# daisy9542/yolo-puncture

Hardware: AMD Instinct MI355X
Metric: images/sec (higher is better)
Workload: dtype bf16

## Files before the change

### include/yolop.h

```cpp
#ifndef YOLOP_H
#define YOLOP_H

#include <stddef.h>
#include <stdint.h>

#ifdef __cplusplus
extern "C" {
#endif

#define YP_OK 0
#define YP_ERR_ARG -1
#define YP_ERR_STATE -2
#define YP_ERR_HIP -3
#define YP_ERR_WEIGHT -4

#define YP_BF16 0
#define YP_F32 1

#define YP_TASK_DETECT 0
#define YP_TASK_SEGMENT 1

#define YP_NM 32
#define YP_MAX_MASKS 480
#define YP_ID_MASKS_FRAMES_BUDGET (1ull << 30)
// ... 121 lines not shown
int yp_tensor_write(yp_engine* e, int tensor, int coff, int C, const float* host);
int yp_tensor_count(const yp_engine* e);
int yp_tensor_info(const yp_engine* e, int i, char* name, int name_cap, int dims[4] , int* is_f32);
int yp_tensor_read(yp_engine* e, int i, float* host_out);

int yp_profile(yp_engine* e, const uint8_t* in_dev, int B, int H, int W, float* det_out, int32_t* idx_out,
               float* coeff_out, float* ms_out, int iters, void* stream);

int yp_set_nms(yp_engine* e, float conf, float iou);

int yp_set_attention_form(yp_engine* e, int form);

int yp_set_attention_f32_stream(yp_engine* e, int on);

int yp_set_autotune(yp_engine* e, int enable);

int yp_tuning_export(const yp_engine* e, int32_t* cfg_out, int cap);
int yp_tuning_import(yp_engine* e, int B, int H, int W, const int32_t* cfg, int n);

int yp_debug_force_conv_cfg(int cfg);
int yp_debug_op_cfg(const yp_engine* e, int i, int* cfg);
int yp_debug_last_store_form(void);
int yp_debug_max_workgroups(int n);
int yp_debug_conv_families(int* base, int* num_cfgs, int cap);
int yp_debug_ablation(int v);
int yp_debug_head_clocks(uint64_t* out8);
int yp_debug_attention(const void* qkv_dev, void* o_dev, int dtype, int B, int N, int nh, int kd, int hd, int q_stride, int q_coff, int o_stride,
                       int o_coff, int wgs, int* kernel_out, void* stream);
int yp_debug_attention_form(const void* qkv_dev, void* o_dev, int dtype, int B, int N, int nh, int kd, int hd, int q_stride, int q_coff, int o_stride,
                            int o_coff, int wgs, int form, int* kernel_out, void* stream);
int yp_debug_attention_f32(const void* qkv_dev, void* o_dev, int B, int N, int nh, int kd, int hd, int q_stride, int q_coff, int o_stride, int o_coff,
                           int wgs, int f32_stream, int* kernel_out, void* stream);
int yp_debug_conv_s2(const void* x_dev, const void* w_dev, const float* bias_dev, const void* res_dev, void* y_dev, int out_f32, int B, int H,
                     int W, int Cin, int Cout, int silu, int cfg, int lds_weights, int64_t* lds_out, char* kernel_out, int kernel_cap,
                     void* stream);
int yp_debug_topk_anchors(const uint32_t* const mk_dev[3], int B, const int hw[3][2], int k, int32_t* sel_out_dev, uint32_t* thr_out_dev, void* stream);
int yp_debug_head_branch_clocks(uint64_t* out8);
int yp_debug_head_winners(yp_engine* e, int32_t* sel_host, float* box_host, float* coeff_host);
int yp_debug_contour_clocks(uint64_t* out12);
int yp_debug_pwsp_clocks(uint64_t* out32);

int yp_tuning_source(const yp_engine* e);

int yp_debug_host_selftest(yp_engine* e);
int yp_debug_graph_info(const yp_engine* e, int64_t* out6);
int yp_debug_head_positions(yp_engine* e, int64_t* out6);
// ... 9 lines not shown
```

### yolo-puncture_amd/csrc/common.h

```cpp
#pragma once
#include <hip/hip_runtime.h>
#include <stdint.h>
#include <atomic>
#include <cstdlib>
#include <initializer_list>
#include <string>
#include <type_traits>
#include <vector>

namespace yp {

enum DType { DT_BF16 = 0, DT_F32 = 1 };
enum Act { ACT_NONE = 0, ACT_SILU = 1, ACT_RELU = 2 };

enum OpKind {
    OP_STEM = 0,
    OP_CONV = 1,
    OP_DWCONV = 2,
    OP_POOL5 = 3,
    OP_UPSAMPLE = 4,
    OP_ATTN = 5,
    OP_HEAD = 6,
    OP_CONVT = 7,
    OP_AMAX = 9,
// ... 106 lines not shown
    void* y; int y_stride, y_coff; int Ho, Wo;
    const void* res; int res_stride, res_coff;
    int B, ks, stride, pad, act;
    int gs, gstride;
    size_t x_bytes;
};

struct StemParams {
    const uint8_t* x; int H, W;
    const float* w;
    const void* wpk;
    const float* bias;
    void* y; int y_stride, y_coff; int Ho, Wo, C0; int B;
    int act;
};

struct FrontParams {
    const uint8_t* img; int imgH, imgW, B;
    const void* w0; const float* bias0; int act0, C0; int H1, W1;
    const void* w1; const float* bias1; int act1, C1, Kpad1; size_t w1_bytes;
    const void* w2; const float* bias2; int act2, C2, Kpad2; size_t w2_bytes;
    void* y; int y_stride, y_coff; size_t y_bytes; int Ho, Wo;
    unsigned long long* clk;
};
bool frontend_valid(const FrontParams& p);
hipError_t launch_frontend(const FrontParams& p, hipStream_t st);

struct C2fParams {
    const void* x; int x_stride, x_coff; size_t x_bytes;
    int B, H, W, C;
    const void* w1; const float* bias1; int act1, Kpad1; size_t w1_bytes;
    const void* w2; const float* bias2; int act2, Kpad2; size_t w2_bytes;
    int shortcut;
    const void* w3; const float* bias3; int act3, Kpad3, Cout; size_t w3_bytes;
    void* y; int y_stride, y_coff; size_t y_bytes;
    unsigned long long* clk;
    int wide;
};
bool c2f_fused_valid(const C2fParams& p);

struct ScdParams {
    const void* x; int x_stride, x_coff; size_t x_bytes; int B, H, W, K;
    const void* w1; const float* bias1; int act1, Kpad1, C; size_t w1_bytes;
    const void* wd; const float* biasd; int actd;
    void* y; int y_stride, y_coff; size_t y_bytes; int Ho, Wo;
    unsigned long long* clk;
};
bool scdown_fused_valid(const ScdParams& p);
// ... 313 lines not shown
```

### yolo-puncture_amd/csrc/engine.hip

```cpp
#include "../../include/yolop.h"
#include "common.h"
#include <algorithm>
#include <array>
#include <chrono>

#include <cmath>
#include <cstdarg>
#include <cstdio>
#include <cstring>
#include <cstdlib>
#include <dlfcn.h>
#include <fcntl.h>
#include <fstream>
#include <map>
#include <sstream>
#include <memory>

using namespace yp;

static thread_local char g_err[512] = "";
static int fail(int code, const char* fmt, ...) {
    va_list ap;
    va_start(ap, fmt);
    vsnprintf(g_err, sizeof(g_err), fmt, ap);
// ... 9 lines not shown

struct yp_engine {
    yp_model_desc desc{};
    int device = 0;
    int dtype = DT_BF16;
    std::vector<TensorDesc> tensors;
    std::vector<WeightDesc> weights;
    std::vector<Op> ops;
    std::map<std::string, int> wmap;
    bool finalized = false;
    int pB = 0, pH = 0, pW = 0;
    bool planned = false, allocated = false;
    void* arena = nullptr;
    size_t arena_bytes = 0;
    int proto_t = -1;
    void* mask_ws = nullptr;
    void* head_ws = nullptr;
    size_t head_ws_bytes = 0;
    size_t mask_ws_bytes = 0;
    bool use_graph = false;
    bool graph_auto = false;
    std::map<std::array<int, 3>, bool> auto_replay;
    bool fuse = true;
    int attn_form = ATTN_FORM_AUTO;
    int attn_f32_stream = ATTN_F32_GENERIC;
    bool tail = false;
    bool narrow_store = false;
    bool sparse_head = true;
    void* sp_ws = nullptr; size_t sp_ws_bytes = 0;
    bool tune = true;
    int tune_source = 0;
    hipStream_t own_stream = nullptr;
    hipEvent_t ev_in = nullptr;
    hipGraphExec_t gexec = nullptr;
    hipGraph_t gsrc = nullptr;
    bool use_lanes = true;
    int n_captures = 0;
    int g_nodes = 0, g_edges = 0, g_edges_expected = 0;
    hipStream_t last_stream = nullptr; bool have_last = false;
    struct LaneStep { int op = -1; std::vector<int> waits; bool fork = false; bool record = false; };
    std::vector<LaneStep> lane_steps;
    std::vector<int> lanes_used;
    int n_lanes = 1;
    bool warmed = false;
    struct Tuned { int cfg; std::string kernel; };
    std::map<std::array<int, 3>, std::vector<Tuned>> tuned;
// ... 587 lines not shown
    p.out_f32 = (to.f32 && e.dtype == DT_BF16) ? 1 : 0;
    p.wide = (e.dtype == DT_BF16 && !p.out_f32 && !e.narrow_store) ? 1 : 0;
    p.up = 1; p.oy = 0; p.ox = 0;
    p.x_bytes = ti.bytes; p.w_bytes = w.mat_bytes; p.y_bytes = to.bytes; p.cfg = o.cfg; p.dbg = conv_debug_ablation();
    if (o.folded) {
        const Op& u = e.ops[o.fold_up];
        const TensorDesc& t2 = e.tensors[u.in.t];
        p.x2 = t2.ptr; p.x2_bytes = t2.bytes; p.x2_stride = t2.C; p.x2_coff = u.in.coff; p.x2_C = u.out.C; p.x2_H = t2.H; p.x2_W = t2.W;
    }
    return p;
}

static FrontParams front_params(const yp_engine& e, const Op& o, const uint8_t* img) {
    const Op& c1 = e.ops[o.fuse_pre];
    const Op& st = e.ops[o.stem_op];
    const WeightDesc &w0 = e.weights[st.widx], &w1 = e.weights[c1.widx], &w2 = e.weights[o.widx];
    const TensorDesc &t0 = e.tensors[st.out.t], &to = e.tensors[o.out.t];
    FrontParams p{};
    p.img = img; p.imgH = e.pH; p.imgW = e.pW; p.B = e.pB;
    p.w0 = w0.d_w2; p.bias0 = w0.d_b; p.act0 = st.act; p.C0 = st.out.C; p.H1 = t0.H; p.W1 = t0.W;
    p.w1 = w1.d_w; p.bias1 = w1.d_b; p.act1 = c1.act; p.C1 = c1.out.C; p.Kpad1 = w1.Kpad; p.w1_bytes = w1.mat_bytes;
    p.w2 = w2.d_w; p.bias2 = w2.d_b; p.act2 = o.act; p.C2 = o.out.C; p.Kpad2 = w2.Kpad; p.w2_bytes = w2.mat_bytes;
    p.y = to.ptr; p.y_stride = to.C; p.y_coff = o.out.coff; p.y_bytes = to.bytes; p.Ho = to.H; p.Wo = to.W;
    return p;
}

static C2fParams c2f_params(const yp_engine& e, const Op& o) {
    const Op &m1 = e.ops[o.c2f_m1], &m2 = e.ops[o.c2f_m2];
    const WeightDesc &w1 = e.weights[m1.widx], &w2 = e.weights[m2.widx], &w3 = e.weights[o.widx];
    const TensorDesc &ti = e.tensors[o.in.t], &to = e.tensors[o.out.t];
    C2fParams p{};
    p.x = ti.ptr; p.x_stride = ti.C; p.x_coff = o.in.coff; p.x_bytes = ti.bytes; p.B = e.pB; p.H = ti.H; p.W = ti.W; p.C = m1.in.C;
    p.w1 = w1.d_w; p.bias1 = w1.d_b; p.act1 = m1.act; p.Kpad1 = w1.Kpad; p.w1_bytes = w1.mat_bytes;
    p.w2 = w2.d_w; p.bias2 = w2.d_b; p.act2 = m2.act; p.Kpad2 = w2.Kpad; p.w2_bytes = w2.mat_bytes;
    p.shortcut = m2.res.t >= 0 ? 1 : 0;
    p.w3 = w3.d_w; p.bias3 = w3.d_b; p.act3 = o.act; p.Kpad3 = w3.Kpad; p.Cout = o.out.C; p.w3_bytes = w3.mat_bytes;
    p.y = to.ptr; p.y_stride = to.C; p.y_coff = o.out.coff; p.y_bytes = to.bytes;
    p.wide = (e.dtype == DT_BF16 && !to.f32 && !e.narrow_store) ? 1 : 0;
    if (m1.in.t != o.in.t || m1.in.coff != o.in.coff + p.C || m2.out.t != o.in.t || m2.out.coff != o.in.coff + 2 * p.C || o.in.C != 3 * p.C ||
        m1.k != 3 || m2.k != 3 || m1.s != 1 || m2.s != 1 || m1.out.C != p.C || m2.out.C != p.C || m1.res.t >= 0 ||
        (m2.res.t >= 0 && (m2.res.t != m1.in.t || m2.res.coff != m1.in.coff)) || (to.f32 && e.dtype == DT_BF16)) p.C = 0;
    return p;
}

static ScdParams scd_params(const yp_engine& e, const Op& o) {
    const Op& c1 = e.ops[o.scd_pre];
// ... 142 lines not shown
static void tail_views(const yp_engine& e, const Op& o, View& in, View& extra) {
    in = e.ops[e.ops[o.fuse_tail].fuse_dw].in;
    if (o.tail_amax >= 0) extra = e.ops[o.tail_amax].out;
}

static int s2pw_absorbed(const yp_engine&, const Op& o, int m[3]) { return link1(o.fuse_pre, m); }
static std::string s2pw_admit(const yp_engine& e, const Op& o, int& cfg) {
    const ConvParams q = conv_params(e, o);
    const int c = conv_halo_s2_pw_cfg(q);
    if (c < 0) return "";
    cfg = conv_halo_s2_family.base + c;
    return conv_halo_s2_family.symbol(q, c);
}
static void s2pw_views(const yp_engine& e, const Op& o, View& in, View&) { in = e.ops[o.fuse_pre].in; }
static hipError_t s2pw_launch(const yp_engine& e, const Op& o, const RunArgs&, hipStream_t st) {
    return conv_halo_s2_family.launch(conv_params(e, o), o.cfg - conv_halo_s2_family.base, st);
}

static int front_absorbed(const yp_engine&, const Op& o, int m[3]) {
    m[0] = o.stem_op; m[1] = o.fuse_pre;
    return o.stem_op >= 0 && o.fuse_pre >= 0 ? 2 : 0;
}
static std::string front_admit(const yp_engine& e, const Op& o, int&) {
    return e.weights[e.ops[o.stem_op].widx].d_w2 && frontend_valid(front_params(e, o, nullptr)) ? "frontend_kernel" : "";
}
static void front_views(const yp_engine&, const Op&, View& in, View&) { in = View{}; }
static hipError_t front_launch(const yp_engine& e, const Op& o, const RunArgs& a, hipStream_t st) { return launch_frontend(front_params(e, o, a.in), st); }

static int c2f_absorbed(const yp_engine&, const Op& o, int m[3]) {
    m[0] = o.c2f_m1; m[1] = o.c2f_m2;
    return o.c2f_m1 >= 0 ? 2 : 0;
}
static std::string c2f_admit(const yp_engine& e, const Op& o, int&) { return c2f_fused_valid(c2f_params(e, o)) ? "c2f_fused_kernel" : ""; }
static void c2f_views(const yp_engine& e, const Op& o, View& in, View&) { in = View{o.in.t, o.in.coff, 2 * e.ops[o.c2f_m1].in.C}; }
static hipError_t c2f_launch(const yp_engine& e, const Op& o, const RunArgs&, hipStream_t st) { return launch_c2f_fused(c2f_params(e, o), st); }

static int scd_absorbed(const yp_engine&, const Op& o, int m[3]) { return link1(o.scd_pre, m); }
static std::string scd_admit(const yp_engine& e, const Op& o, int&) {
    const ScdParams q = scd_params(e, o);
    return scdown_fused_valid(q) ? scdown_fused_kernel_name(q) : "";
}
static void scd_views(const yp_engine& e, const Op& o, View& in, View&) { in = e.ops[o.scd_pre].in; }
static hipError_t scd_launch(const yp_engine& e, const Op& o, const RunArgs&, hipStream_t st) { return launch_scdown_fused(scd_params(e, o), st); }

static int pwsp_absorbed(const yp_engine&, const Op& o, int m[3]) { return link1(o.pw_pre, m); }
static std::string pwsp_admit(const yp_engine& e, const Op& o, int&) {
    const PwSpParams q = pwsp_params(e, o);
// ... 913 lines not shown
        memset(&sa, 0, sizeof(sa));
        sa.sa_handler = yp_fatal_handler;
        sigemptyset(&sa.sa_mask);
        sa.sa_flags = SA_NODEFER | SA_ONSTACK;
        if (sigaction(g_fatal_sigs[i], &sa, &g_prev_sa[i]) != 0) g_prev_sa[i].sa_handler = SIG_DFL;
    }
}

static_assert(YP_MAX_DET == HEAD_MAXK, "include/yolop.h promises what the head kernels hold (head_select.h MAXK, head_nms_common.h NMAXK)");

int yp_create(const yp_model_desc* desc, int device, yp_engine** out) {
    if (!desc || !out) return fail(YP_ERR_ARG, "null argument");
    if (desc->nc <= 0 || desc->max_det <= 0) return fail(YP_ERR_ARG, "bad nc/max_det");
    if (desc->max_det > YP_MAX_DET)
        return fail(YP_ERR_ARG, "max_det = %d: the head kernels rank at most %d rows per image (max_det <= %d)", desc->max_det, YP_MAX_DET, YP_MAX_DET);
    if (desc->task == YP_TASK_SEGMENT && desc->max_det > YP_MAX_MASKS)
        return fail(YP_ERR_ARG, "segmentation engines take max_det <= %d (the mask tail keeps one frame's coefficients in LDS; ultralytics' default is 300)", YP_MAX_MASKS);
    if (desc->dtype != YP_BF16 && desc->dtype != YP_F32) return fail(YP_ERR_ARG, "bad dtype");
    if (desc->task != YP_TASK_DETECT && desc->task != YP_TASK_SEGMENT) return fail(YP_ERR_ARG, "bad task");
    install_fatal_handlers();
    std::unique_ptr<yp_engine> e(new yp_engine());
    e->desc = *desc; e->device = device; e->dtype = desc->dtype;
    e->fuse = !env_on("YOLOP_NO_FUSE");
    e->tail = env_on("YOLOP_TAIL");
    if (const char* v = std::getenv("YOLOP_ATTN_FORM")) {
        if (!strcmp(v, "stream")) e->attn_form = ATTN_FORM_STREAM;
        else if (!strcmp(v, "stream_wide")) e->attn_form = ATTN_FORM_STREAM_WIDE;
        else if (*v && strcmp(v, "auto")) return fail(YP_ERR_ARG, "YOLOP_ATTN_FORM=%s (auto | stream | stream_wide)", v);
    }
    if (const char* v = std::getenv("YOLOP_ATTN_F32")) {
        if (!strcmp(v, "stream")) e->attn_f32_stream = ATTN_F32_STREAM;
        else if (!strcmp(v, "stream_wide")) e->attn_f32_stream = ATTN_F32_STREAM_WIDE;
        else if (*v) return fail(YP_ERR_ARG, "YOLOP_ATTN_F32=%s (stream | stream_wide, or unset)", v);
    }
    e->sparse_head = !env_on("YOLOP_DENSE_HEAD");
    e->narrow_store = env_on("YOLOP_NARROW_STORE");
    int rc = build_graph(*e);
    if (rc != YP_OK) return rc;
    for (const Op& o : e->ops)
        for (const View* v : {&o.in, &o.out, &o.res})
            if (v->t >= 0 && o.kind != OP_STEM && ((v->C & 7) || (v->coff & 7)) && !e->tensors[v->t].f32)
                return fail(YP_ERR_ARG, "op %s: channel slice (%d,%d) is not a multiple of 8", o.name.c_str(), v->coff, v->C);
    *out = e.release();
    return YP_OK;
}

// ... 648 lines not shown
int yp_debug_contour_clocks(uint64_t* out12) {
    if (!out12) return fail(YP_ERR_ARG, "yp_debug_contour_clocks: null output");
    HIPCHK(hipDeviceSynchronize());
    HIPCHK(contour_read_clocks((unsigned long long*)out12));
    return YP_OK;
}

int yp_debug_ablation(int v) {
    conv_set_debug_ablation(v);
    return 0;
}

int yp_debug_force_conv_cfg(int cfg) {
    conv_dma_force_cfg(cfg);
    return conv_dma_family.num_cfgs;
}

int yp_debug_last_store_form(void) {
    store_form_watched().store(true);
    return last_store_form().exchange(-1);
}

int yp_debug_max_workgroups(int n) { return debug_max_workgroups_ref().exchange(n > 0 ? n : 0); }

int yp_debug_op_cfg(const yp_engine* e, int i, int* cfg) {
    if (!e || i < 0 || i >= (int)e->ops.size() || !cfg) return fail(YP_ERR_ARG, "bad argument");
    *cfg = op_launch_cfg(*e, e->ops[i]);
    return YP_OK;
}

int yp_debug_conv_families(int* base, int* num_cfgs, int cap) {
    for (int f = 0; f < kNumConvFamilies && f < cap; ++f) {
        if (base) base[f] = kConvFamilies[f]->base;
        if (num_cfgs) num_cfgs[f] = kConvFamilies[f]->num_cfgs;
    }
    return kNumConvFamilies;
}

int yp_debug_host_selftest(yp_engine* e) {
    if (!e) return fail(YP_ERR_ARG, "null engine");
    if (!e->planned) return fail(YP_ERR_STATE, "yp_plan has not been called");
    size_t acc = 0;
    if (!e->finalized)
        for (WeightDesc& w : e->weights) {
            if (!w.have_w || !w.have_b || w.w.empty()) continue;
            std::vector<unsigned char> main, aux;
// ... 378 lines not shown
```

### yolo-puncture_amd/csrc/frontend.hip

```cpp
#include "common.h"
#include <cstdio>
#include <cstdlib>
#include <vector>
#include <type_traits>

namespace yp {

constexpr int FE_TH = 8;
constexpr int FE_HR = 2 * FE_TH + 1;
constexpr int FE_HP = FE_HR * 33;
constexpr int FE_HPAD = 576;
constexpr int FE_HB = 36 * 1024;
constexpr int FE_NW = 8;

struct FeRows { unsigned d[3][3]; };

__device__ __forceinline__ void fe_load(const FrontParams& p, const __amdgpu_buffer_rsrc_t irs, int b, int sy, int sx, bool live, FeRows& r) {
    const int rowbytes = p.imgW * 3;
    const int ab = ((sx * 2 - 1) * 3) & ~3;
#pragma unroll
    for (int ky = 0; ky < 3; ++ky) {
        const int hi = sy * 2 - 1 + ky;
        const bool rok = live && (unsigned)hi < (unsigned)p.imgH;
        const int base = (b * p.imgH + hi) * rowbytes + ab;
#pragma unroll
        for (int k = 0; k < 3; ++k) {
            const int off = base + 4 * k;
            r.d[ky][k] = __builtin_amdgcn_raw_buffer_load_b32(irs, (rok && off >= 0) ? (unsigned)off : kBufferOOB, 0, 0);
        }
    }
}

__device__ __forceinline__ void fe_row(const FeRows& r, int sx, unsigned char* dst, int hp) {
    __attribute__((aligned(16))) __bf16 row[32];
#pragma unroll
    for (int i = 27; i < 32; ++i) row[i] = (__bf16)0.f;
    const int sb = (sx * 2 - 1) * 3;
    const unsigned sbytes = (unsigned)(sb - (sb & ~3));
    const float k = 1.0f / 255.0f;
#pragma unroll
    for (int ky = 0; ky < 3; ++ky) {
        unsigned w0 = __builtin_amdgcn_alignbyte(r.d[ky][1], r.d[ky][0], sbytes);
        const unsigned w1 = __builtin_amdgcn_alignbyte(r.d[ky][2], r.d[ky][1], sbytes);
        const unsigned w2 = __builtin_amdgcn_alignbyte(0u, r.d[ky][2], sbytes);
        if (sx == 0) w0 &= 0xff000000u;
        __bf16* rr = row + ky * 9;
        rr[0] = (__bf16)((float)(w0 & 0xffu) * k);          rr[1] = (__bf16)((float)((w0 >> 8) & 0xffu) * k);
        rr[2] = (__bf16)((float)((w0 >> 16) & 0xffu) * k);  rr[3] = (__bf16)((float)(w0 >> 24) * k);
        rr[4] = (__bf16)((float)(w1 & 0xffu) * k);          rr[5] = (__bf16)((float)((w1 >> 8) & 0xffu) * k);
        rr[6] = (__bf16)((float)((w1 >> 16) & 0xffu) * k);  rr[7] = (__bf16)((float)(w1 >> 24) * k);
        rr[8] = (__bf16)((float)(w2 & 0xffu) * k);
    }
    const uint4* r4 = (const uint4*)row;
#pragma unroll
    for (int c = 0; c < 4; ++c) *(uint4*)(dst + hp * 64 + ((c ^ cswz64(hp)) * 16)) = r4[c];
}

__global__ __launch_bounds__(FE_NW * 64) void frontend_kernel(const FrontParams p, const int tiles_h, const int tiles_w, const int G) {
    constexpr int FM = 2, FN = 2, WGM = 4;
    constexpr int BN = 64;
    extern __shared__ __attribute__((aligned(1024))) unsigned char smem[];
    unsigned char* const Hs = smem;
    unsigned char* const Ib = Hs + FE_HB;
    unsigned char* const W1s = Ib + FE_HB;
    unsigned char* const W2s = W1s + 9 * BN * 64;
    unsigned char* const W0s = W2s + BN * 128;
    unsigned char* const Vs = W0s + 32 * 64;

    const int tid = threadIdx.x, lane = tid & 63;
    const int wave = __builtin_amdgcn_readfirstlane(tid >> 6);
    const int wm = wave % WGM, wn = wave / WGM;
    const int fr = lane & 15, fc = lane >> 4;
    const int num_tiles = p.B * tiles_h * tiles_w;

    const int bid = xcd_remap(blockIdx.x, gridDim.x);

// ... 205 lines not shown
                for (int r = 0; r < FM; ++r) acc[a][r] = __builtin_amdgcn_mfma_f32_16x16x32_bf16(w2f[a], t2f[r], acc[a][r], 0, 0, 0);
        }
        const int wo = tw * 16 + fr;
#pragma unroll
        for (int r = 0; r < FM; ++r) {
            const int ho = th * FE_TH + wm * FM + r;
            const bool pix_ok = (ho < p.Ho) && (wo < p.Wo);
            const unsigned m = (unsigned)((b * p.Ho + ho) * p.Wo + wo);
#pragma unroll
            for (int a = 0; a < FN; ++a) {
                const int co = wn * (FN * 16) + a * 16 + fc * 4;
                float v[4] = {acc[a][r][0], acc[a][r][1], acc[a][r][2], acc[a][r][3]};
                if (p.act2 == ACT_SILU) silu4_packed(v);
                const unsigned off = pix_ok ? (m * (unsigned)p.y_stride + (unsigned)(p.y_coff + co)) * 2u : kBufferOOB;
                store_bf16x4(v, yrs, off);
            }
        }
        FE_STAMP(4)
    }
    if (p.clk && lane == 0)
        for (int i = 0; i < 6; ++i) p.clk[((size_t)blockIdx.x * FE_NW + wave) * 6 + i] = clk[i];
}

static size_t frontend_lds() { return (size_t)2 * FE_HB + 9 * 64 * 64 + 64 * 128 + 32 * 64 + 1024; }

bool frontend_valid(const FrontParams& p) {
    if (p.C0 != 32 || p.C1 != 64 || p.C2 != 64 || p.Kpad1 != 9 * 32 || p.Kpad2 != 64) return false;
    if ((p.imgH & 3) || (p.imgW & 3) || p.H1 * 2 != p.imgH || p.W1 * 2 != p.imgW || p.Ho * 2 != p.H1 || p.Wo * 2 != p.W1) return false;
    if ((p.y_stride & 3) || (p.y_coff & 3) || p.y_bytes >= (1ull << 31)) return false;
    if ((long)p.B * p.imgH * p.imgW * 3 >= (1l << 31)) return false;
    const long covered = (long)((p.Ho + FE_TH - 1) / FE_TH * FE_TH) * ((p.Wo + 15) / 16 * 16);
    if (covered * 2 > (long)p.Ho * p.Wo * 3) return false;
    return true;
}

hipError_t launch_frontend(const FrontParams& p, hipStream_t st) {
    const size_t sh = frontend_lds();
    const int tiles_h = (p.Ho + FE_TH - 1) / FE_TH, tiles_w = (p.Wo + 15) / 16;
    const int num_tiles = p.B * tiles_h * tiles_w;
    int G = 256;
    if (G > num_tiles) G = num_tiles;
    static size_t granted = 0;
    if (hipError_t e = allow_dynamic_lds((const void*)frontend_kernel, sh, granted)) return e;
    static const bool clocks = env_on("YOLOP_FRONT_CLOCKS");
    if (clocks) {
        FrontParams q = p;
        const size_t n = (size_t)G * FE_NW * 6;
        if (hipMalloc((void**)&q.clk, n * 8) != hipSuccess) return hipErrorOutOfMemory;
        hipLaunchKernelGGL(frontend_kernel, dim3(G), dim3(FE_NW * 64), sh, st, q, tiles_h, tiles_w, G);
        (void)hipStreamSynchronize(st);
        std::vector<unsigned long long> h(n);
        (void)hipMemcpy(h.data(), q.clk, n * 8, hipMemcpyDeviceToHost);
        (void)hipFree(q.clk);
        static const char* nm[6] = {"A im2col", "B stem", "C 3x3s2", "D silu->lds", "E 1x1+store", "barriers"};
        const double tiles_per = (double)num_tiles / G;
        for (int w = 0; w < FE_NW; w += FE_NW - 1) {
            fprintf(stderr, "[frontend clocks] wave %d, s_memtime ticks per tile:", w);
            for (int i = 0; i < 6; ++i) {
                double s = 0;
                for (int g = 0; g < G; ++g) s += (double)h[((size_t)g * FE_NW + w) * 6 + i];
                fprintf(stderr, " %s %.0f", nm[i], s / G / tiles_per);
            }
            fprintf(stderr, "\n");
        }
        return hipGetLastError();
    }
    hipLaunchKernelGGL(frontend_kernel, dim3(G), dim3(FE_NW * 64), sh, st, p, tiles_h, tiles_w, G);
    return hipGetLastError();
}

}
```

### yolo-puncture_amd/engine.py

```python
from __future__ import annotations

import ctypes as C
import os
from typing import Dict, List, Optional, Tuple

import numpy as np
import torch

from .weights import fold_state

_LIB: Optional[C.CDLL] = None
_HERE = os.path.dirname(os.path.abspath(__file__))
LIB_PATH = os.environ.get("YOLOP_LIB") or os.path.join(_HERE, "libyolop.so")

YP_BF16, YP_F32 = 0, 1
TASK_DETECT, TASK_SEGMENT = 0, 1
OP_KINDS = {0: "stem", 1: "conv", 2: "dwconv", 3: "pool5", 4: "upsample", 5: "attn", 6: "head", 7: "convT", 8: "pool3", 9: "amax"}
FORMS = ("plain", "dwpw", "dwpw_tail", "s2pw", "frontend", "c2f", "scdown", "pwsp", "cls_out")


class ModelDesc(C.Structure):
    _fields_ = [("variant", C.c_int), ("nc", C.c_int), ("task", C.c_int), ("dtype", C.c_int), ("max_det", C.c_int), ("family", C.c_int)]


# ... 63 lines not shown
    lib.yp_tensor_read.argtypes = [vp, C.c_int, vp]
    lib.yp_profile.argtypes = [vp, vp, C.c_int, C.c_int, C.c_int, vp, vp, vp, vp, C.c_int, vp]
    lib.yp_set_graph.argtypes = [vp, C.c_int]
    lib.yp_set_autotune.argtypes = [vp, C.c_int]
    lib.yp_set_nms.argtypes = [vp, C.c_float, C.c_float]
    lib.yp_set_nms.restype = C.c_int
    lib.yp_debug_host_selftest.argtypes = [vp]
    lib.yp_debug_host_selftest.restype = C.c_int
    lib.yp_tuning_source.argtypes = [vp]
    lib.yp_tuning_source.restype = C.c_int
    lib.yp_debug_graph_info.argtypes = [vp, C.POINTER(C.c_int64)]
    lib.yp_debug_graph_info.restype = C.c_int
    lib.yp_debug_head_positions.argtypes = [vp, C.POINTER(C.c_int64)]
    lib.yp_debug_head_positions.restype = C.c_int
    lib.yp_debug_marker.argtypes = [vp]
    lib.yp_debug_marker.restype = C.c_int
    lib.yp_debug_force_conv_cfg.argtypes = [C.c_int]
    lib.yp_debug_op_cfg.argtypes = [vp, C.c_int, ip]
    lib.yp_debug_op_cfg.restype = C.c_int
    lib.yp_debug_last_store_form.argtypes = []
    lib.yp_debug_last_store_form.restype = C.c_int
    lib.yp_debug_max_workgroups.argtypes = [C.c_int]
    lib.yp_debug_max_workgroups.restype = C.c_int
    lib.yp_debug_conv_families.argtypes = [ip, ip, C.c_int]
    lib.yp_debug_conv_families.restype = C.c_int
    lib.yp_debug_ablation.argtypes = [C.c_int]
    lib.yp_debug_head_clocks.argtypes = [C.POINTER(C.c_uint64)]
    lib.yp_debug_head_branch_clocks.argtypes = [C.POINTER(C.c_uint64)]
    lib.yp_debug_contour_clocks.argtypes = [C.POINTER(C.c_uint64)]
    lib.yp_debug_pwsp_clocks.argtypes = [C.POINTER(C.c_uint64)]
    lib.yp_letterbox.argtypes = [vp, C.c_int, C.c_int, vp] + [C.c_int] * 7 + [vp]
    lib.yp_letterbox.restype = C.c_int
    lib.yp_letterbox_batch.argtypes = [vp, C.c_int, C.c_int, C.c_int, vp] + [C.c_int] * 7 + [vp]
    lib.yp_letterbox_batch.restype = C.c_int
    lib.yp_masks_frames.argtypes = [vp, vp, C.c_int, vp, C.c_long, vp, C.c_int, C.c_int, vp, vp]
    lib.yp_masks_frames.restype = C.c_int
    lib.yp_masks_frames_input.argtypes = [vp, vp, C.c_int, vp, C.c_long, vp, C.c_int, C.c_int, vp, vp]
    lib.yp_masks_frames_input.restype = C.c_int
    lib.yp_id_masks_frames.argtypes = [vp, vp, vp, C.c_int, vp, vp, C.c_int, C.c_int, C.c_int, C.c_int, vp, vp, C.c_int, C.c_int, vp]
    lib.yp_id_masks_frames.restype = C.c_int
    lib.yp_id_masks_frames_workspace.argtypes = [vp] + [C.c_int] * 6
    lib.yp_id_masks_frames_workspace.restype = C.c_size_t
    lib.yp_comm_unique_id.argtypes = [vp]
    lib.yp_comm_create.argtypes = [vp, C.c_int, C.c_int, C.c_int, C.POINTER(vp)]
    lib.yp_allgather.argtypes = [vp, vp, vp, C.c_size_t, vp]
    lib.yp_comm_destroy.argtypes = [vp]
    for fn in ("yp_comm_unique_id", "yp_comm_create", "yp_allgather", "yp_comm_destroy"):
        getattr(lib, fn).restype = C.c_int
    for fn in ("yp_create", "yp_destroy", "yp_weight_count", "yp_weight_info", "yp_set_weight", "yp_finalize",
               "yp_forward", "yp_proto", "yp_masks", "yp_plan", "yp_op_info", "yp_op_output", "yp_op_input", "yp_tensor_count",
               "yp_tensor_info", "yp_tensor_read", "yp_profile", "yp_set_graph", "yp_run_op", "yp_tensor_write",
               "yp_op_kernel", "yp_set_autotune", "yp_debug_force_conv_cfg", "yp_debug_ablation"):
        getattr(lib, fn).restype = C.c_int
    if path is None:
        _LIB = lib
    return lib


EXPORTS = ["yp_last_error", "yp_create", "yp_destroy", "yp_weight_count", "yp_weight_info", "yp_set_weight",
           "yp_finalize", "yp_forward", "yp_proto", "yp_masks", "yp_id_mask_resized", "yp_plan", "yp_op_info", "yp_op_output", "yp_op_input", "yp_op_fusion",
           "yp_tensor_count", "yp_tensor_info", "yp_tensor_read", "yp_profile", "yp_set_graph", "yp_run_op",
           "yp_tensor_write", "yp_op_kernel", "yp_set_autotune", "yp_tuning_export", "yp_tuning_import", "yp_set_nms", "yp_debug_force_conv_cfg", "yp_debug_op_cfg", "yp_debug_op_form", "yp_debug_last_store_form", "yp_debug_max_workgroups", "yp_debug_conv_families", "yp_debug_ablation", "yp_debug_head_clocks", "yp_debug_head_branch_clocks", "yp_debug_head_winners", "yp_debug_contour_clocks", "yp_debug_pwsp_clocks", "yp_debug_host_selftest", "yp_debug_graph_info", "yp_tuning_source", "yp_debug_head_positions", "yp_debug_marker", "yp_max_batch", "yp_debug_topk_anchors", "yp_debug_attention", "yp_debug_attention_form", "yp_debug_attention_f32", "yp_debug_conv_s2", "yp_set_attention_form", "yp_set_attention_f32_stream", "yp_letterbox", "yp_letterbox_batch", "yp_masks_frames", "yp_masks_frames_input", "yp_id_masks_frames", "yp_id_masks_frames_workspace", "yp_mask_contours",
           "yp_mask_contours_scaled", "yp_mask_contours_large_workspace", "yp_mask_contours_large", "yp_comm_unique_id", "yp_comm_create", "yp_allgather", "yp_comm_destroy",
           "yp_u2net_create", "yp_u2net_destroy", "yp_u2net_weight_count", "yp_u2net_weight_info", "yp_u2net_set_weight", "yp_u2net_finalize",
           "yp_u2net_forward", "yp_u2net_forward_crops", "yp_u2net_set_graph", "yp_u2net_tensor_count", "yp_u2net_tensor_info", "yp_u2net_tensor_read",
           "yp_u2net_op_count", "yp_u2net_op_info",
           "yp_cls_create", "yp_cls_destroy", "yp_cls_weight_count", "yp_cls_weight_info", "yp_cls_set_weight", "yp_cls_finalize",
           "yp_cls_forward", "yp_cls_set_graph", "yp_cls_tensor_count", "yp_cls_tensor_info", "yp_cls_tensor_read"]


MAX_ANCHORS = 294912
MAX_MASKS = 480
ID_MASKS_FRAMES_BUDGET = 1 << 30
ATTENTION_FORMS = {"auto": 0, "stream": 1, "stream_wide": 3}


ATTENTION_F32 = {"generic": 0, "stream": 1}
ATTENTION_F32_WIDE = {"stream_wide": 3}


def _attention_f32(value) -> int:
    if value in ATTENTION_F32:
        return ATTENTION_F32[value]
    if value in ATTENTION_F32_WIDE:
        return ATTENTION_F32_WIDE[value]
# ... 562 lines not shown
```

Before: 23330.

## Add 4-wave register-pipelined frontend kernel with two resident workgroups per CU

Adds a new fused frontend kernel (stem + 3x3s2 conv + 1x1 conv) that uses 4 waves and a smaller LDS footprint. It builds the stem operand in registers via permlane swaps instead of an LDS im2col, prefetches the next tile's image rows into registers during the current tile, and reuses wave-private halo rows for the 1x1 operand. The goal is to fit two workgroups per CU and overlap image loads with compute, launching twice as many workgroups. This becomes the default when occupancy allows; the old phased kernel remains behind an env var and as a fallback. The risk is higher register pressure and more complex lane-transposition logic.

```diff
diff --git a/include/yolop.h b/include/yolop.h
--- a/include/yolop.h
+++ b/include/yolop.h
@@ -167,6 +167,7 @@
 int yp_debug_op_cfg(const yp_engine* e, int i, int* cfg);
 int yp_debug_last_store_form(void);
 int yp_debug_max_workgroups(int n);
+int yp_debug_frontend_query(int phased, int B, int imgH, int imgW, int* lds_bytes);
 int yp_debug_conv_families(int* base, int* num_cfgs, int cap);
 int yp_debug_ablation(int v);
 int yp_debug_head_clocks(uint64_t* out8);
diff --git a/yolo-puncture_amd/csrc/common.h b/yolo-puncture_amd/csrc/common.h
--- a/yolo-puncture_amd/csrc/common.h
+++ b/yolo-puncture_amd/csrc/common.h
@@ -152,8 +152,11 @@
     const void* w2; const float* bias2; int act2, C2, Kpad2; size_t w2_bytes;
     void* y; int y_stride, y_coff; size_t y_bytes; int Ho, Wo;
     unsigned long long* clk;
+    int phased;
 };
 bool frontend_valid(const FrontParams& p);
+size_t frontend_lds(bool phased);
+const char* frontend_kernel_name(const FrontParams& p);
 hipError_t launch_frontend(const FrontParams& p, hipStream_t st);
 
 struct C2fParams {
diff --git a/yolo-puncture_amd/csrc/engine.hip b/yolo-puncture_amd/csrc/engine.hip
--- a/yolo-puncture_amd/csrc/engine.hip
+++ b/yolo-puncture_amd/csrc/engine.hip
@@ -55,6 +55,7 @@
     bool graph_auto = false;
     std::map<std::array<int, 3>, bool> auto_replay;
     bool fuse = true;
+    bool front_phased = false;
     int attn_form = ATTN_FORM_AUTO;
     int attn_f32_stream = ATTN_F32_GENERIC;
     bool tail = false;
@@ -688,6 +689,7 @@
     p.w1 = w1.d_w; p.bias1 = w1.d_b; p.act1 = c1.act; p.C1 = c1.out.C; p.Kpad1 = w1.Kpad; p.w1_bytes = w1.mat_bytes;
     p.w2 = w2.d_w; p.bias2 = w2.d_b; p.act2 = o.act; p.C2 = o.out.C; p.Kpad2 = w2.Kpad; p.w2_bytes = w2.mat_bytes;
     p.y = to.ptr; p.y_stride = to.C; p.y_coff = o.out.coff; p.y_bytes = to.bytes; p.Ho = to.H; p.Wo = to.W;
+    p.phased = e.front_phased ? 1 : 0;
     return p;
 }
 
@@ -876,7 +878,8 @@
     return o.stem_op >= 0 && o.fuse_pre >= 0 ? 2 : 0;
 }
 static std::string front_admit(const yp_engine& e, const Op& o, int&) {
-    return e.weights[e.ops[o.stem_op].widx].d_w2 && frontend_valid(front_params(e, o, nullptr)) ? "frontend_kernel" : "";
+    const FrontParams p = front_params(e, o, nullptr);
+    return e.weights[e.ops[o.stem_op].widx].d_w2 && frontend_valid(p) ? frontend_kernel_name(p) : "";
 }
 static void front_views(const yp_engine&, const Op&, View& in, View&) { in = View{}; }
 static hipError_t front_launch(const yp_engine& e, const Op& o, const RunArgs& a, hipStream_t st) { return launch_frontend(front_params(e, o, a.in), st); }
@@ -1836,6 +1839,7 @@
     std::unique_ptr<yp_engine> e(new yp_engine());
     e->desc = *desc; e->device = device; e->dtype = desc->dtype;
     e->fuse = !env_on("YOLOP_NO_FUSE");
+    e->front_phased = env_on("YOLOP_FRONT_PHASED");
     e->tail = env_on("YOLOP_TAIL");
     if (const char* v = std::getenv("YOLOP_ATTN_FORM")) {
         if (!strcmp(v, "stream")) e->attn_form = ATTN_FORM_STREAM;
@@ -2530,6 +2534,18 @@
 }
 
 int yp_debug_max_workgroups(int n) { return debug_max_workgroups_ref().exchange(n > 0 ? n : 0); }
+
+int yp_debug_frontend_query(int phased, int B, int imgH, int imgW, int* lds_bytes) {
+    FrontParams p{};
+    p.imgH = imgH; p.imgW = imgW; p.B = B; p.phased = phased ? 1 : 0;
+    p.C0 = 32; p.H1 = imgH / 2; p.W1 = imgW / 2;
+    p.C1 = 64; p.Kpad1 = 9 * 32;
+    p.C2 = 64; p.Kpad2 = 64;
+    p.Ho = imgH / 4; p.Wo = imgW / 4; p.y_stride = 64; p.y_coff = 0;
+    p.y_bytes = B > 0 && p.Ho > 0 && p.Wo > 0 ? (size_t)B * p.Ho * p.Wo * 64 * 2 : 0;
+    if (lds_bytes) *lds_bytes = (int)frontend_lds(phased != 0);
+    return B > 0 && imgH > 0 && imgW > 0 && frontend_valid(p) ? 1 : 0;
+}
 
 int yp_debug_op_cfg(const yp_engine* e, int i, int* cfg) {
     if (!e || i < 0 || i >= (int)e->ops.size() || !cfg) return fail(YP_ERR_ARG, "bad argument");
diff --git a/yolo-puncture_amd/csrc/frontend.hip b/yolo-puncture_amd/csrc/frontend.hip
--- a/yolo-puncture_amd/csrc/frontend.hip
+++ b/yolo-puncture_amd/csrc/frontend.hip
@@ -31,7 +31,22 @@
     }
 }
 
-__device__ __forceinline__ void fe_row(const FeRows& r, int sx, unsigned char* dst, int hp) {
+__device__ __forceinline__ void fe_load2(const FrontParams& p, const __amdgpu_buffer_rsrc_t irs, int b, int sy, int sx, bool live, FeRows& r) {
+    const int rowbytes = p.imgW * 3;
+    const int ab = ((sx * 2 - 1) * 3) & ~3;
+#pragma unroll
+    for (int ky = 0; ky < 3; ++ky) {
+        const int hi = sy * 2 - 1 + ky;
+        const bool rok = live && (unsigned)hi < (unsigned)p.imgH;
+        const int base = (b * p.imgH + hi) * rowbytes + ab;
+        const unsigned v1 = rok ? (unsigned)(base + 4) : kBufferOOB;
+        r.d[ky][0] = __builtin_amdgcn_raw_buffer_load_b32(irs, (rok && base >= 0) ? (unsigned)base : kBufferOOB, 0, 0);
+        r.d[ky][1] = __builtin_amdgcn_raw_buffer_load_b32(irs, v1, 0, 0);
+        r.d[ky][2] = __builtin_amdgcn_raw_buffer_load_b32(irs, v1 + 4u, 0, 0);
+    }
+}
+
+__device__ __forceinline__ void fe_row_regs(const FeRows& r, int sx, uint4* out) {
     __attribute__((aligned(16))) __bf16 row[32];
 #pragma unroll
     for (int i = 27; i < 32; ++i) row[i] = (__bf16)0.f;
@@ -52,6 +67,41 @@
         rr[8] = (__bf16)((float)(w2 & 0xffu) * k);
     }
     const uint4* r4 = (const uint4*)row;
+#pragma unroll
+    for (int c = 0; c < 4; ++c) out[c] = r4[c];
+}
+
+__device__ __forceinline__ void fe_row_regs_pk(const FeRows& r, int sx, uint4* out) {
+    typedef __attribute__((ext_vector_type(2))) __bf16 bf16x2;
+    float f[28];
+    f[27] = 0.f;
+    const int sb = (sx * 2 - 1) * 3;
+    const unsigned sbytes = (unsigned)(sb - (sb & ~3));
+    const float k = 1.0f / 255.0f;
+#pragma unroll
+    for (int ky = 0; ky < 3; ++ky) {
+        unsigned w0 = __builtin_amdgcn_alignbyte(r.d[ky][1], r.d[ky][0], sbytes);
+        const unsigned w1 = __builtin_amdgcn_alignbyte(r.d[ky][2], r.d[ky][1], sbytes);
+        const unsigned w2 = __builtin_amdgcn_alignbyte(0u, r.d[ky][2], sbytes);
+        if (sx == 0) w0 &= 0xff000000u;
+        float* ff = f + ky * 9;
+        ff[0] = (float)(w0 & 0xffu) * k;          ff[1] = (float)((w0 >> 8) & 0xffu) * k;
+        ff[2] = (float)((w0 >> 16) & 0xffu) * k;  ff[3] = (float)(w0 >> 24) * k;
+        ff[4] = (float)(w1 & 0xffu) * k;          ff[5] = (float)((w1 >> 8) & 0xffu) * k;
+        ff[6] = (float)((w1 >> 16) & 0xffu) * k;  ff[7] = (float)(w1 >> 24) * k;
+        ff[8] = (float)(w2 & 0xffu) * k;
+    }
+    unsigned d[16];
+#pragma unroll
+    for (int i = 0; i < 14; ++i) d[i] = __builtin_bit_cast(unsigned, __builtin_convertvector(f32x2{f[2 * i], f[2 * i + 1]}, bf16x2));
+    d[14] = 0u; d[15] = 0u;
+#pragma unroll
+    for (int c = 0; c < 4; ++c) out[c] = make_uint4(d[4 * c], d[4 * c + 1], d[4 * c + 2], d[4 * c + 3]);
+}
+
+__device__ __forceinline__ void fe_row(const FeRows& r, int sx, unsigned char* dst, int hp) {
+    uint4 r4[4];
+    fe_row_regs(r, sx, r4);
 #pragma unroll
     for (int c = 0; c < 4; ++c) *(uint4*)(dst + hp * 64 + ((c ^ cswz64(hp)) * 16)) = r4[c];
 }
@@ -303,7 +353,267 @@
         for (int i = 0; i < 6; ++i) p.clk[((size_t)blockIdx.x * FE_NW + wave) * 6 + i] = clk[i];
 }
 
-static size_t frontend_lds() { return (size_t)2 * FE_HB + 9 * 64 * 64 + 64 * 128 + 32 * 64 + 1024; }
+constexpr int FW_NW = 4;
+constexpr int FW_CLK = 8;
+constexpr int FW_NFR = FE_HPAD / 16 / FW_NW;
+constexpr int FW_LDS = FE_HB + 9 * 64 * 64 + 1024;
+static_assert(FW_NFR == 9 && 3 * 33 * 64 >= 32 * 128, "fragment rounds / the wave-private rows hold the 1x1's operand");
+
+template <int NF> __device__ __forceinline__ void fe_transpose(const uint4* row, bf16x8* xf) {
+    const unsigned x[4][4] = {{row[0].x, row[0].y, row[0].z, row[0].w}, {row[1].x, row[1].y, row[1].z, row[1].w},
+                              {row[2].x, row[2].y, row[2].z, row[2].w}, {row[3].x, row[3].y, row[3].z, row[3].w}};
+    u32x4 y[4];
+#pragma unroll
+    for (int d = 0; d < 4; ++d) {
+        const auto lo = __builtin_amdgcn_permlane32_swap(x[0][d], x[2][d], false, false);
+        const auto hi = __builtin_amdgcn_permlane32_swap(x[1][d], x[3][d], false, false);
+        const auto a = __builtin_amdgcn_permlane16_swap(lo[0], hi[0], false, false);
+        const auto b = __builtin_amdgcn_permlane16_swap(lo[1], hi[1], false, false);
+        y[0][d] = a[0]; y[1][d] = a[1]; y[2][d] = b[0]; y[3][d] = b[1];
+    }
+#pragma unroll
+    for (int j = 0; j < NF; ++j) xf[j] = __builtin_bit_cast(bf16x8, y[j]);
+}
+
+__global__ __launch_bounds__(FW_NW * 64, 2) void frontend_kernel_w4(const FrontParams p, const int tiles_h, const int tiles_w, const int G) {
+    constexpr int FM = 2, FN = 4;
+    constexpr int BN = 64;
+    extern __shared__ __attribute__((aligned(1024))) unsigned char smem[];
+    unsigned char* const Hs = smem;
+    unsigned char* const W1s = Hs + FE_HB;
+
+    const int tid = threadIdx.x, lane = tid & 63;
+    const int wave = __builtin_amdgcn_readfirstlane(tid >> 6);
+    const int fr = lane & 15, fc = lane >> 4;
+    unsigned char* const Ds = Hs + (4 * wave + 1) * 33 * 64;
+    float* const Bs = (float*)(W1s + 9 * BN * 64);
+    const int num_tiles = p.B * tiles_h * tiles_w;
+
+    const int bid = xcd_remap(blockIdx.x, gridDim.x);
+
+    const __amdgpu_buffer_rsrc_t w1rs = __builtin_amdgcn_make_buffer_rsrc((void*)p.w1, 0, (int)p.w1_bytes, 0x00020000);
+    const __amdgpu_buffer_rsrc_t w2rs = __builtin_amdgcn_make_buffer_rsrc((void*)p.w2, 0, (int)p.w2_bytes, 0x00020000);
+    const __amdgpu_buffer_rsrc_t w0rs = __builtin_amdgcn_make_buffer_rsrc((void*)p.w0, 0, 32 * 32 * 2, 0x00020000);
+    const __amdgpu_buffer_rsrc_t yrs = __builtin_amdgcn_make_buffer_rsrc((void*)p.y, 0, (int)p.y_bytes, 0x00020000);
+    const __amdgpu_buffer_rsrc_t irs = __builtin_amdgcn_make_buffer_rsrc((void*)p.img, 0, (int)((long)p.B * p.imgH * p.imgW * 3), 0x00020000);
+
+    for (int ii = wave; ii < 9 * BN * 64 / 1024; ii += FW_NW) {
+        const int s = ii * 64 + lane;
+        const int rg = s >> 2, pc = s & 3;
+        const int c8 = pc ^ cswz64(rg);
+        const int n = rg % BN, tap = rg / BN;
+        const unsigned voff = (unsigned)((n * p.Kpad1 + tap * 32 + c8 * 8) * 2);
+        __builtin_amdgcn_raw_ptr_buffer_load_lds(w1rs, (lds_void*)(W1s + ii * 1024), 16, voff, 0, 0, 0);
+    }
+    bf16x8 w2f[2][FN], w0f[2];
+#pragma unroll
+    for (int ss = 0; ss < 2; ++ss)
+#pragma unroll
+        for (int a = 0; a < FN; ++a)
+            w2f[ss][a] = __builtin_bit_cast(bf16x8, __builtin_amdgcn_raw_buffer_load_b128(w2rs, (unsigned)(((a * 16 + fr) * p.Kpad2 + (ss * 4 + fc) * 8) * 2), 0, 0));
+#pragma unroll
+    for (int h = 0; h < 2; ++h) w0f[h] = __builtin_bit_cast(bf16x8, __builtin_amdgcn_raw_buffer_load_b128(w0rs, (unsigned)(((h * 16 + fr) * 32 + fc * 8) * 2), 0, 0));
+
+    if (tid < 64) { Bs[tid] = p.bias1[tid]; Bs[64 + tid] = p.bias2[tid]; }
+    if (tid < 32) Bs[128 + tid] = p.bias0[tid];
+
+    auto patch_rc = [](int hp, int& jr, int& jc) {
+        jr = hp / 33;
+        const int e = hp - jr * 33;
+        jc = (e < 17) ? 2 * e : 2 * (e - 17) + 1;
+    };
+    int bjr[3], bjc[3];
+    bool bok[3];
+#pragma unroll
+    for (int q = 0; q < 3; ++q) {
+        const int hp = (wave * FW_NFR + 4 * q) * 16 + lane;
+        bok[q] = hp < FE_HP && (q < 2 || lane < 16);
+        patch_rc(hp, bjr[q], bjc[q]);
+    }
+    int crc[FW_NFR];
+#pragma unroll
+    for (int f = 0; f < FW_NFR; ++f) {
+        const int hp = (wave * FW_NFR + f) * 16 + fr;
+        int jr, jc;
+        patch_rc(hp, jr, jc);
+        crc[f] = hp < FE_HP ? (jr | (jc << 8)) : -1;
+    }
+    auto tile_pos = [&](int tile, int& b, int& th, int& tw) {
+        int t = tile;
+        tw = t % tiles_w; t /= tiles_w;
+        th = t % tiles_h;
+        b = t / tiles_h;
+    };
+    FeRows rr[3];
+#pragma unroll
+    for (int k = 0; k < 3; ++k) { rr[2].d[k][0] = 0u; rr[2].d[k][1] = 0u; rr[2].d[k][2] = 0u; }
+    auto prefetch = [&](int tile, int q) {
+        int b, th, tw;
+        tile_pos(tile, b, th, tw);
+        const int sy = 2 * th * FE_TH - 1 + bjr[q], sx = 2 * tw * 16 - 1 + bjc[q];
+        const bool live = tile < num_tiles && bok[q] && (unsigned)sy < (unsigned)p.H1 && (unsigned)sx < (unsigned)p.W1;
+        if (q < 2 || lane < 16) fe_load2(p, irs, b, sy, sx, live, rr[q]);
+    };
+    int tile = bid;
+#pragma unroll
+    for (int q = 0; q < 3; ++q) prefetch(tile, q);
+
+    __builtin_amdgcn_s_waitcnt(0 | (7 << 4) | (0xF << 8));
+    asm volatile("s_waitcnt lgkmcnt(0)" ::: "memory");
+    __builtin_amdgcn_s_barrier();
+
+    unsigned long long clk[6] = {0, 0, 0, 0, 0, 0};
+    unsigned long long last = p.clk ? __builtin_amdgcn_s_memtime() : 0ull;
+    const unsigned long long t_begin = last;
+    for (; tile < num_tiles; tile += G) {
+        int b, th, tw;
+        tile_pos(tile, b, th, tw);
+        const int sy0 = 2 * th * FE_TH - 1, sx0 = 2 * tw * 16 - 1;
+        auto stem_round = [&](auto NFC, auto QC) {
+            constexpr int NF = decltype(NFC)::value, q = decltype(QC)::value;
+            uint4 row[4];
+            fe_row_regs_pk(rr[q], sx0 + bjc[q], row);
+            bf16x8 xf[NF];
+            fe_transpose<NF>(row, xf);
+            prefetch(tile + G, q);
+            float4 bias0[2];
+            bias0[0] = *(const float4*)(Bs + 128 + fc * 4);
+            bias0[1] = *(const float4*)(Bs + 128 + 16 + fc * 4);
+            FE_STAMP(0)
+            f32x4 acc[NF][2];
+#pragma unroll
+            for (int j = 0; j < NF; ++j)
+#pragma unroll
+                for (int h = 0; h < 2; ++h) {
+                    acc[j][h] = f32x4{bias0[h].x, bias0[h].y, bias0[h].z, bias0[h].w};
+                    acc[j][h] = __builtin_amdgcn_mfma_f32_16x16x32_bf16(w0f[h], xf[j], acc[j][h], 0, 0, 0);
+                }
+#pragma unroll
+            for (int j = 0; j < NF; ++j) {
+                const int rc = crc[4 * q + j];
+                const int hp = (wave * FW_NFR + 4 * q + j) * 16 + fr;
+                const int sy = sy0 + (rc & 0xff), sx = sx0 + (rc >> 8);
+                const bool in = rc >= 0 && (unsigned)sy < (unsigned)p.H1 && (unsigned)sx < (unsigned)p.W1;
+#pragma unroll
+                for (int h = 0; h < 2; ++h) {
+                    __attribute__((aligned(8))) __bf16 o[4];
+                    float sv[4] = {acc[j][h][0], acc[j][h][1], acc[j][h][2], acc[j][h][3]};
+                    if (p.act0 == ACT_SILU) silu4_packed(sv);
+#pragma unroll
+                    for (int i = 0; i < 4; ++i) o[i] = (__bf16)(in ? sv[i] : 0.f);
+                    if (rc >= 0) *(uint2*)(Hs + hp * 64 + (((2 * h + (fc >> 1)) ^ cswz64(hp)) * 16) + (fc & 1) * 8) = *(const uint2*)o;
+                }
+            }
+            FE_STAMP(1)
+        };
+        stem_round(std::integral_constant<int, 4>{}, std::integral_constant<int, 0>{});
+        stem_round(std::integral_constant<int, 4>{}, std::integral_constant<int, 1>{});
+        stem_round(std::integral_constant<int, 1>{}, std::integral_constant<int, 2>{});
+        asm volatile("s_waitcnt lgkmcnt(0)" ::: "memory");
+        FE_STAMP(1)
+        __builtin_amdgcn_s_barrier();
+        FE_STAMP(5)
+        f32x4 acc[FN][FM];
+#pragma unroll
+        for (int a = 0; a < FN; ++a)
+#pragma unroll
+            for (int r = 0; r < FM; ++r) acc[a][r] = *(const f32x4*)(Bs + a * 16 + fc * 4);
+#pragma unroll
+        for (int kx = 0; kx < 3; ++kx) {
+            bf16x8 wf[3][FN];
+#pragma unroll
+            for (int ky = 0; ky < 3; ++ky)
+#pragma unroll
+                for (int a = 0; a < FN; ++a) {
+                    const int rw = (ky * 3 + kx) * BN + a * 16 + fr;
+                    wf[ky][a] = *(const bf16x8*)(W1s + swz64((unsigned)(rw * 64 + fc * 16)));
+                }
+            const int eoff = (kx == 1) ? 17 + fr : fr + (kx >> 1);
+#pragma unroll
+            for (int jj = 0; jj < 2 * FM + 1; ++jj) {
+                const int hp = (2 * wave * FM + jj) * 33 + eoff;
+                const bf16x8 xf = *(const bf16x8*)(Hs + swz64((unsigned)(hp * 64 + fc * 16)));
+                if (jj & 1) {
+#pragma unroll
+                    for (int a = 0; a < FN; ++a) acc[a][jj >> 1] = __builtin_amdgcn_mfma_f32_16x16x32_bf16(wf[1][a], xf, acc[a][jj >> 1], 0, 0, 0);
+                } else {
+                    if ((jj >> 1) < FM) {
+#pragma unroll
+                        for (int a = 0; a < FN; ++a) acc[a][jj >> 1] = __builtin_amdgcn_mfma_f32_16x16x32_bf16(wf[0][a], xf, acc[a][jj >> 1], 0, 0, 0);
+                    }
+                    if ((jj >> 1) >= 1) {
+#pragma unroll
+                        for (int a = 0; a < FN; ++a)
+                            acc[a][(jj >> 1) - 1] = __builtin_amdgcn_mfma_f32_16x16x32_bf16(wf[2][a], xf, acc[a][(jj >> 1) - 1], 0, 0, 0);
+                    }
+                }
+            }
+        }
+        asm volatile("" ::: "memory");
+        FE_STAMP(2)
+#pragma unroll
+        for (int r = 0; r < FM; ++r) {
+            const int px = r * 16 + fr;
+#pragma unroll
+            for (int a = 0; a < FN; ++a) {
+                const int co = a * 16 + fc * 4;
+                __attribute__((aligned(8))) __bf16 o[4];
+                float sv[4] = {acc[a][r][0], acc[a][r][1], acc[a][r][2], acc[a][r][3]};
+                if (p.act1 == ACT_SILU) silu4_packed(sv);
+#pragma unroll
+                for (int i = 0; i < 4; ++i) o[i] = (__bf16)sv[i];
+                *(uint2*)(Ds + px * 128 + (((co >> 3) ^ ((px >> 1) & 7)) * 16) + (co & 7) * 2) = *(const uint2*)o;
+            }
+        }
+        asm volatile("" ::: "memory");
+        FE_STAMP(3)
+        bf16x8 t2f[2][FM];
+#pragma unroll
+        for (int ss = 0; ss < 2; ++ss)
+#pragma unroll
+            for (int r = 0; r < FM; ++r) {
+                const int px = r * 16 + fr;
+                t2f[ss][r] = *(const bf16x8*)(Ds + px * 128 + (((ss * 4 + fc) ^ ((px >> 1) & 7)) * 16));
+            }
+        asm volatile("s_waitcnt lgkmcnt(0)" ::: "memory");
+        FE_STAMP(4)
+        __builtin_amdgcn_s_barrier();
+        FE_STAMP(5)
+#pragma unroll
+        for (int a = 0; a < FN; ++a)
+#pragma unroll
+            for (int r = 0; r < FM; ++r) acc[a][r] = *(const f32x4*)(Bs + 64 + a * 16 + fc * 4);
+#pragma unroll
+        for (int ss = 0; ss < 2; ++ss)
+#pragma unroll
+            for (int a = 0; a < FN; ++a)
+#pragma unroll
+                for (int r = 0; r < FM; ++r) acc[a][r] = __builtin_amdgcn_mfma_f32_16x16x32_bf16(w2f[ss][a], t2f[ss][r], acc[a][r], 0, 0, 0);
+        const int wo = tw * 16 + fr;
+#pragma unroll
+        for (int r = 0; r < FM; ++r) {
+            const int ho = th * FE_TH + wave * FM + r;
+            const bool pix_ok = (ho < p.Ho) && (wo < p.Wo);
+            const unsigned m = (unsigned)((b * p.Ho + ho) * p.Wo + wo);
+#pragma unroll
+            for (int a = 0; a < FN; ++a) {
+                const int co = a * 16 + fc * 4;
+                float v[4] = {acc[a][r][0], acc[a][r][1], acc[a][r][2], acc[a][r][3]};
+                if (p.act2 == ACT_SILU) silu4_packed(v);
+                const unsigned off = pix_ok ? (m * (unsigned)p.y_stride + (unsigned)(p.y_coff + co)) * 2u : kBufferOOB;
+                store_bf16x4(v, yrs, off);
+            }
+        }
+        FE_STAMP(4)
+    }
+    if (p.clk && lane == 0) {
+        unsigned long long* const c = p.clk + ((size_t)blockIdx.x * FW_NW + wave) * FW_CLK;
+        for (int i = 0; i < 6; ++i) c[i] = clk[i];
+        c[6] = t_begin; c[7] = last;
+    }
+}
+
+size_t frontend_lds(bool phased) { return phased ? (size_t)2 * FE_HB + 9 * 64 * 64 + 64 * 128 + 32 * 64 + 1024 : (size_t)FW_LDS; }
 
 bool frontend_valid(const FrontParams& p) {
     if (p.C0 != 32 || p.C1 != 64 || p.C2 != 64 || p.Kpad1 != 9 * 32 || p.Kpad2 != 64) return false;
@@ -315,38 +625,71 @@
     return true;
 }
 
+static int frontend_w4_resident() {
+    static const int n = [] {
+        static size_t granted = 0;
+        int r = 0;
+        if (allow_dynamic_lds((const void*)frontend_kernel_w4, (size_t)FW_LDS, granted) != hipSuccess) return 0;
+        if (hipOccupancyMaxActiveBlocksPerMultiprocessor(&r, (const void*)frontend_kernel_w4, FW_NW * 64, (size_t)FW_LDS) != hipSuccess) { (void)hipGetLastError(); return 0; }
+        return r;
+    }();
+    return n;
+}
+static bool frontend_runs_phased(const FrontParams& p) { return p.phased || frontend_w4_resident() < 2; }
+
+const char* frontend_kernel_name(const FrontParams& p) { return frontend_runs_phased(p) ? "frontend_kernel" : "frontend_kernel_w4"; }
+
 hipError_t launch_frontend(const FrontParams& p, hipStream_t st) {
-    const size_t sh = frontend_lds();
+    const bool phased = frontend_runs_phased(p);
+    const auto kern = phased ? frontend_kernel : frontend_kernel_w4;
+    const int nw = phased ? FE_NW : FW_NW;
+    const size_t sh = frontend_lds(phased);
     const int tiles_h = (p.Ho + FE_TH - 1) / FE_TH, tiles_w = (p.Wo + 15) / 16;
     const int num_tiles = p.B * tiles_h * tiles_w;
-    int G = 256;
+    int G = phased ? 256 : 2 * 256;
     if (G > num_tiles) G = num_tiles;
-    static size_t granted = 0;
-    if (hipError_t e = allow_dynamic_lds((const void*)frontend_kernel, sh, granted)) return e;
+    if (const int cap = debug_max_workgroups()) G = G < cap ? G : cap;
+    static size_t granted[2] = {0, 0};
+    if (hipError_t e = allow_dynamic_lds((const void*)kern, sh, granted[phased ? 0 : 1])) return e;
     static const bool clocks = env_on("YOLOP_FRONT_CLOCKS");
     if (clocks) {
         FrontParams q = p;
-        const size_t n = (size_t)G * FE_NW * 6;
+        const int nc = phased ? 6 : FW_CLK;
+        const size_t n = (size_t)G * nw * nc;
         if (hipMalloc((void**)&q.clk, n * 8) != hipSuccess) return hipErrorOutOfMemory;
-        hipLaunchKernelGGL(frontend_kernel, dim3(G), dim3(FE_NW * 64), sh, st, q, tiles_h, tiles_w, G);
+        hipLaunchKernelGGL(kern, dim3(G), dim3(nw * 64), sh, st, q, tiles_h, tiles_w, G);
         (void)hipStreamSynchronize(st);
         std::vector<unsigned long long> h(n);
         (void)hipMemcpy(h.data(), q.clk, n * 8, hipMemcpyDeviceToHost);
         (void)hipFree(q.clk);
         static const char* nm[6] = {"A im2col", "B stem", "C 3x3s2", "D silu->lds", "E 1x1+store", "barriers"};
         const double tiles_per = (double)num_tiles / G;
-        for (int w = 0; w < FE_NW; w += FE_NW - 1) {
+        for (int w = 0; w < nw; w += nw - 1) {
             fprintf(stderr, "[frontend clocks] wave %d, s_memtime ticks per tile:", w);
             for (int i = 0; i < 6; ++i) {
                 double s = 0;
-                for (int g = 0; g < G; ++g) s += (double)h[((size_t)g * FE_NW + w) * 6 + i];
+                for (int g = 0; g < G; ++g) s += (double)h[((size_t)g * nw + w) * nc + i];
                 fprintf(stderr, " %s %.0f", nm[i], s / G / tiles_per);
             }
             fprintf(stderr, "\n");
         }
+        if (!phased) {
+            fprintf(stderr, "[frontend clocks] loop ticks of the slowest workgroup per XCD:");
+            for (int x = 0; x < 8 && x < G; ++x) {
+                double hi = 0, sum = 0;
+                int cnt = 0;
+                for (int g = x; g < G; g += 8) {
+                    const unsigned long long* c = &h[((size_t)g * nw) * nc];
+                    const double d = (double)(c[7] - c[6]);
+                    hi = d > hi ? d : hi; sum += d; ++cnt;
+                }
+                fprintf(stderr, " %.0f (mean %.0f)", hi, sum / cnt);
+            }
+            fprintf(stderr, "\n");
+        }
         return hipGetLastError();
     }
-    hipLaunchKernelGGL(frontend_kernel, dim3(G), dim3(FE_NW * 64), sh, st, p, tiles_h, tiles_w, G);
+    hipLaunchKernelGGL(kern, dim3(G), dim3(nw * 64), sh, st, p, tiles_h, tiles_w, G);
     return hipGetLastError();
 }
 
diff --git a/yolo-puncture_amd/engine.py b/yolo-puncture_amd/engine.py
--- a/yolo-puncture_amd/engine.py
+++ b/yolo-puncture_amd/engine.py
@@ -109,6 +109,8 @@
     lib.yp_debug_last_store_form.restype = C.c_int
     lib.yp_debug_max_workgroups.argtypes = [C.c_int]
     lib.yp_debug_max_workgroups.restype = C.c_int
+    lib.yp_debug_frontend_query.argtypes = [C.c_int, C.c_int, C.c_int, C.c_int, ip]
+    lib.yp_debug_frontend_query.restype = C.c_int
     lib.yp_debug_conv_families.argtypes = [ip, ip, C.c_int]
     lib.yp_debug_conv_families.restype = C.c_int
     lib.yp_debug_ablation.argtypes = [C.c_int]
@@ -147,7 +149,7 @@
 EXPORTS = ["yp_last_error", "yp_create", "yp_destroy", "yp_weight_count", "yp_weight_info", "yp_set_weight",
            "yp_finalize", "yp_forward", "yp_proto", "yp_masks", "yp_id_mask_resized", "yp_plan", "yp_op_info", "yp_op_output", "yp_op_input", "yp_op_fusion",
            "yp_tensor_count", "yp_tensor_info", "yp_tensor_read", "yp_profile", "yp_set_graph", "yp_run_op",
-           "yp_tensor_write", "yp_op_kernel", "yp_set_autotune", "yp_tuning_export", "yp_tuning_import", "yp_set_nms", "yp_debug_force_conv_cfg", "yp_debug_op_cfg", "yp_debug_op_form", "yp_debug_last_store_form", "yp_debug_max_workgroups", "yp_debug_conv_families", "yp_debug_ablation", "yp_debug_head_clocks", "yp_debug_head_branch_clocks", "yp_debug_head_winners", "yp_debug_contour_clocks", "yp_debug_pwsp_clocks", "yp_debug_host_selftest", "yp_debug_graph_info", "yp_tuning_source", "yp_debug_head_positions", "yp_debug_marker", "yp_max_batch", "yp_debug_topk_anchors", "yp_debug_attention", "yp_debug_attention_form", "yp_debug_attention_f32", "yp_debug_conv_s2", "yp_set_attention_form", "yp_set_attention_f32_stream", "yp_letterbox", "yp_letterbox_batch", "yp_masks_frames", "yp_masks_frames_input", "yp_id_masks_frames", "yp_id_masks_frames_workspace", "yp_mask_contours",
+           "yp_tensor_write", "yp_op_kernel", "yp_set_autotune", "yp_tuning_export", "yp_tuning_import", "yp_set_nms", "yp_debug_force_conv_cfg", "yp_debug_op_cfg", "yp_debug_op_form", "yp_debug_last_store_form", "yp_debug_max_workgroups", "yp_debug_frontend_query", "yp_debug_conv_families", "yp_debug_ablation", "yp_debug_head_clocks", "yp_debug_head_branch_clocks", "yp_debug_head_winners", "yp_debug_contour_clocks", "yp_debug_pwsp_clocks", "yp_debug_host_selftest", "yp_debug_graph_info", "yp_tuning_source", "yp_debug_head_positions", "yp_debug_marker", "yp_max_batch", "yp_debug_topk_anchors", "yp_debug_attention", "yp_debug_attention_form", "yp_debug_attention_f32", "yp_debug_conv_s2", "yp_set_attention_form", "yp_set_attention_f32_stream", "yp_letterbox", "yp_letterbox_batch", "yp_masks_frames", "yp_masks_frames_input", "yp_id_masks_frames", "yp_id_masks_frames_workspace", "yp_mask_contours",
            "yp_mask_contours_scaled", "yp_mask_contours_large_workspace", "yp_mask_contours_large", "yp_comm_unique_id", "yp_comm_create", "yp_allgather", "yp_comm_destroy",
            "yp_u2net_create", "yp_u2net_destroy", "yp_u2net_weight_count", "yp_u2net_weight_info", "yp_u2net_set_weight", "yp_u2net_finalize",
            "yp_u2net_forward", "yp_u2net_forward_crops", "yp_u2net_set_graph", "yp_u2net_tensor_count", "yp_u2net_tensor_info", "yp_u2net_tensor_read",
```

New measurement: 23420, median of 6. About the same (+0.4%).
